# apple/ml-pgdvs

Measured on AMD Instinct MI355X. Metric: novel-view frames/s at 1080p x 24 src frames; achieved HBM GB/s vs gfx950 peak, higher is better.
Workload: dtype f32

## Files before the change

### ml-pgdvs_amd/csrc/fused.h

```cpp
#pragma once
#include "common.h"

namespace pgdvs {

struct WarpExtras {
  uint8_t *zero_a, *zero_b;
  uint4 *zero0, *zero1, *zero2, *zero3;
  int n16_0, n16_1, n16_2, n16_3;
  int32_t *chunk_cnt;
};
int dyn_warp_fused(int H, int W, const float *dyn_mask1, const float *occ, int use_flow_consistency, const float *flow12,
                   const float *depth1, const float *depth2, const float *rgb1, const float *rgb2, const float *cam1,
                   const float *cam2, const float *times, uint8_t *mask_eff, uint8_t *valid, float *pcl, float *rgbf,
                   const WarpExtras &ex, hipStream_t st);

int compact_gather_bbox(const uint8_t *flags, int64_t n, const int32_t *chunk_cnt, int32_t *idx_out, int32_t *count_out,
                        const float *rows_in, float *rows_out, unsigned *bbox, int32_t *zero_per_row, int zero_mult, hipStream_t st);

void knn_grid_state_block(void *workspace, int64_t capacity, void **block, int64_t *bytes, unsigned **bbox, void **tab,
                          int64_t *tab_bytes, int32_t **occ_count, int *occ_mult, void **coarse, int64_t *coarse_bytes);
int knn_grid_mean_dist_prepared(const float *pts, const int32_t *count, int64_t capacity, int K, float *avg_out, void *workspace,
                                int64_t workspace_bytes, hipStream_t st);

void outlier_hist_block(void *workspace, void **block, int64_t *bytes);
int outlier_keep_fused(const float *avg, const int32_t *count, int64_t capacity, float std_thres, float *thres_out,
                       const int32_t *idx, uint8_t *keep, void *workspace, int64_t workspace_bytes, hipStream_t st);

int dyn_splat_scatter_part_fused(int H, int W, const float *rgb1, const float *rgb2, const float *flow12, const float *cam_tgt,
                                 const float *pcl, const uint8_t *keep, float *flow_1_to_tgt, float *valid_mask,
                                 const float *noise, const unsigned long long *rng, float alpha, void *workspace,
                                 bool flags_cleared, hipStream_t st);
uint8_t *dyn_splat_flag_map(void *workspace, int H, int W);


void raster_counter_block(void *workspace, int64_t n_rows, int H, int W, float radius, void **block, int64_t *bytes);
int points_raster_bounded_cleared(const float *pts, int64_t pts_stride, const float *feat, int64_t feat_stride, int64_t n_points,
                                  const int64_t *n_points_dev, int64_t row_bound, int32_t *status_dev, const float *cam_tgt,
                                  float radius, int K, int H, int W, float *rgb, int rgb_planar, float *mask, void *workspace,
                                  int64_t workspace_bytes, pgdvs_stream_t stream, bool counters_cleared);

}
```

### ml-pgdvs_amd/csrc/raster.hip

```cpp
#include <cstdlib>

#include "common.h"
#include "raster_cam.h"
#include "wave.h"

namespace pgdvs {

constexpr int kTile = 16;

struct TileBox {
  int tx0, tx1, ty0, ty1;
};

__device__ __forceinline__ TileBox tile_box(const RasterCam &rc, float3 p, float radius, int H,
                                            int W, int ntx, int nty) {
  TileBox b;
  b.tx0 = 1;
  b.tx1 = 0;
  b.ty0 = 1;
  b.ty1 = 0;
  if (!(p.z >= 0.0f) || !isfinite(p.x) || !isfinite(p.y)) return b;
  float offx = rc.range_x / 2.0f, offy = rc.range_y / 2.0f;
  float xc = (float)(W - 1) - ((p.x + offx) * (float)W - offx) / rc.range_x;
  float yc = (float)(H - 1) - ((p.y + offy) * (float)H - offy) / rc.range_y;
  float rpx = radius * (float)W / rc.range_x + 0.0625f;
  float rpy = radius * (float)H / rc.range_y + 0.0625f;
  float x0 = ceilf(xc - rpx), x1 = floorf(xc + rpx);
  float y0 = ceilf(yc - rpy), y1 = floorf(yc + rpy);
  if (x1 < x0 || y1 < y0) return b;
  if (x1 < 0.0f || y1 < 0.0f || x0 > (float)(W - 1) || y0 > (float)(H - 1)) return b;
  int ix0 = x0 < 0.0f ? 0 : (int)x0, iy0 = y0 < 0.0f ? 0 : (int)y0;
  int ix1 = x1 > (float)(W - 1) ? W - 1 : (int)x1, iy1 = y1 > (float)(H - 1) ? H - 1 : (int)y1;
  b.tx0 = ix0 / kTile;
  b.tx1 = ix1 / kTile;
  b.ty0 = iy0 / kTile;
  b.ty1 = iy1 / kTile;
// ... 131 lines not shown
    b.tx0 = 1; b.tx1 = 0; b.ty0 = 1; b.ty1 = 0;
    float pz = 0.0f;
    if (i < n) {
      float3 p = point_to_ndc(rc, cur[0], cur[1], cur[2]);
      b = tile_box(rc, p, radius, H, W, ntx, nty);
      pz = p.z + 0.0f;
    }
    int nx = 2, ny = 2;
    if (!box2) {
      nx = wave_max_i32_scalar(b.tx1 - b.tx0 + 1);
      ny = wave_max_i32_scalar(b.ty1 - b.ty0 + 1);
    }
    for (int jy = 0; jy < ny; ++jy)
      for (int jx = 0; jx < nx; ++jx) {
        int tx = b.tx0 + jx, ty = b.ty0 + jy;
        int t = (tx <= b.tx1 && ty <= b.ty1) ? ty * ntx + tx : -1;
        if (tile_bound != nullptr && t >= 0 && pz > tile_bound[t]) t = -1;
        if (local)
          wave_tile_count_lds(s_tab, t);
        else
          wave_tile_count(tile_count, t);
      }
  }
  if (local) {
    __syncthreads();
    for (int t = threadIdx.x; t < ntiles; t += kBinThreads) {
      const int v = s_tab[t];
      if (v) __hip_atomic_fetch_add(&tile_count[t], v, __ATOMIC_RELAXED, __HIP_MEMORY_SCOPE_AGENT);
    }
  }
}

__global__ void __launch_bounds__(1024)
raster_scan_kernel(const int32_t *__restrict__ counts, int n, int32_t *__restrict__ offsets, const int32_t *__restrict__ run_flag) {
  __shared__ int wave_sums[1024 / kWave];
  if (run_flag != nullptr && *run_flag == 0) return;
  constexpr int kPer = 8;
  const int lane = threadIdx.x & 63, wave = threadIdx.x >> 6;
  int carry = 0;
  for (int start = 0; start < n; start += 1024 * kPer) {
    const int i0 = start + (int)threadIdx.x * kPer;
    int v[kPer], s = 0;
#pragma unroll
    for (int k = 0; k < kPer; ++k) {
      v[k] = i0 + k < n ? counts[i0 + k] : 0;
      s += v[k];
    }
    const int x = wave_incl_scan(s);
    if (lane == 63) wave_sums[wave] = x;
    __syncthreads();
    int run = carry + x - s, total = 0;
#pragma unroll
    for (int w = 0; w < 1024 / kWave; ++w) {
      if (w < wave) run += wave_sums[w];
      total += wave_sums[w];
    }
#pragma unroll
    for (int k = 0; k < kPer; ++k) {
      if (i0 + k < n) offsets[i0 + k] = run;
      run += v[k];
    }
    carry += total;
    __syncthreads();
  }
  if (threadIdx.x == 0) offsets[n] = carry;
}

constexpr int kFillPer = 4;
// ... 211 lines not shown
#pragma unroll
    for (int k = 0; k < K - 1; ++k) c[k] = kk < key[k];
    c[K - 1] = true;
#pragma unroll
    for (int k = K - 1; k > 0; --k) key[k] = c[k - 1] ? key[k - 1] : (c[k] ? kk : key[k]);
    key[0] = c[0] ? kk : key[0];
  }
};

constexpr int kSortCap = 2048;
constexpr int kSortCapLong = 4096;
constexpr int kSortBuckets = 1024;
constexpr int kSortMaxBucket = 64;

template <int K>
__device__ __forceinline__ void rank_insert(float (&key)[K], float r) {
#pragma unroll
  for (int k = K - 1; k > 0; --k) key[k] = __builtin_amdgcn_fmed3f(key[k - 1], key[k], r);
  asm("v_min_f32 %0, %1, %2" : "=v"(key[0]) : "v"(key[0]), "v"(r));
}

__device__ __forceinline__ float readlane_f(float v, int lane) {
  return __int_as_float(__builtin_amdgcn_readlane(__float_as_int(v), lane));
}

template <int K, int kCap, bool kFrag>
__global__ void __launch_bounds__(256, kCap <= kSortCap ? (kFrag ? 4 : 5) : 2)
raster_tile_kernel(const float4 *__restrict__ lists, const int32_t *__restrict__ offsets, int64_t list_capacity,
                   const float4 *__restrict__ seg_lists, const int32_t *__restrict__ seg_count, int seg,
                   const int32_t *__restrict__ seg_overflow, int pass,
                   const float *__restrict__ feat, int64_t feat_stride, float radius, int H, int W,
                   int ntx, int nty, int tiles_per_xcd, int64_t *__restrict__ idx_out,
                   float *__restrict__ zbuf_out, float *__restrict__ dist_out,
                   float *__restrict__ rgb_out, int rgb_planar, float *__restrict__ mask_out, int32_t *__restrict__ stats) {
  constexpr int kSortPerThread = kCap / 256;
  __shared__ uint2 s_buf[kCap];
  uint2 *s_kz = s_buf;
  float2 *s_xy = reinterpret_cast<float2 *>(s_buf);
  __shared__ unsigned s_id[kCap];
  __shared__ unsigned s_zr[kFrag ? kCap : 1];
  __shared__ float4 s_wave[4][68];
  unsigned *s_cnt = reinterpret_cast<unsigned *>(&s_wave[0][0]);
  static_assert(kSortBuckets * 4 <= 4 * 68 * 16, "the counters alias the strips");
  static_assert(kCap * (kFrag ? 16 : 12) + 4 * 68 * 16 + 128 <= (kCap <= kSortCap ? (kFrag ? 40960 : 32768) : 81920),
                "four / five (two) workgroups per CU");
  static_assert(kCap % 256 == 0 && kCap <= 4096, "every thread owns kCap / 256 entries; positions are packed in 12 bits");
  __shared__ unsigned s_red[12];
  __shared__ int s_flag;
  const int ntiles = ntx * nty;
  (void)tiles_per_xcd;
  const int tile = blockIdx.x;
  if (tile >= ntiles) return;
  const int ty = tile / ntx, tx = tile - ty * ntx;
  const int tid = threadIdx.x, lane = tid & 63, wave = tid >> 6;
  const int lx = (wave & 1) * 8 + (lane & 7), ly = (wave >> 1) * 8 + (lane >> 3);
  const int xi = tx * kTile + lx, yi = ty * kTile + ly;
  const bool inside = xi < W && yi < H;
  const float range_x = W > H ? 2.0f * (float)W / (float)H : 2.0f;
  const float range_y = H > W ? 2.0f * (float)H / (float)W : 2.0f;
  const float xf = inside ? pix_to_ndc(W - 1 - xi, W, range_x) : __builtin_nanf("");
  const float yf = pix_to_ndc(H - 1 - yi, H, range_y);
  const float r2 = radius * radius;
  const int qx0 = tx * kTile + (wave & 1) * 8, qy0 = ty * kTile + (wave >> 1) * 8;
  const float margin = radius * 1.001f + 1e-6f;
  const float bx_hi = pix_to_ndc(W - 1 - qx0, W, range_x) + margin;
  const float bx_lo = pix_to_ndc(W - 1 - (qx0 + 7), W, range_x) - margin;
  const float by_hi = pix_to_ndc(H - 1 - qy0, H, range_y) + margin;
// ... 272 lines not shown
  const size_t pix = (size_t)yi * W + xi;
  float t = 0.0f;
#pragma unroll
  for (int k = 0; k < K; ++k)
    if (has[k]) t = t + (1.0f - rd2[k] / r2);
  t = t > 1e-4f ? t : 1e-4f;
  float acc[3] = {0.f, 0.f, 0.f}, ones = 0.0f;
#pragma unroll
  for (int k = 0; k < K; ++k) {
    if (idx_out) idx_out[pix * K + k] = has[k] ? (int64_t)rid[k] : (int64_t)-1;
    if (zbuf_out) zbuf_out[pix * K + k] = has[k] ? rz[k] : -1.0f;
    if (dist_out) dist_out[pix * K + k] = rd2[k];
    if (has[k]) {
      float w = 1.0f - rd2[k] / r2;
      ones = ones + w * 1.0f / t;
      if (rgb_out) {
        const float *f = feat + (int64_t)rid[k] * feat_stride;
#pragma unroll
        for (int c = 0; c < 3; ++c) acc[c] = acc[c] + w * f[c] / t;
      }
    }
  }
  if (rgb_out) {
    if (rgb_planar) {
      const size_t P = (size_t)H * W;
#pragma unroll
      for (int c = 0; c < 3; ++c) rgb_out[c * P + pix] = acc[c];
    } else {
#pragma unroll
      for (int c = 0; c < 3; ++c) rgb_out[pix * 3 + c] = acc[c];
    }
  }
  if (mask_out) mask_out[pix] = ones > 0.0f ? 1.0f : 0.0f;
}

__global__ void raster_status_kernel(const int64_t *__restrict__ n_dev, int32_t *__restrict__ status) {
  if (threadIdx.x == 0) *status = (n_dev && *n_dev > 0) ? 1 : ((n_dev && *n_dev < 0) ? 2 : 0);
}

static int64_t max_tiles_per_point(float radius, int H, int W) {
  float range_x = W > H ? 2.0f * (float)W / (float)H : 2.0f;
  float range_y = H > W ? 2.0f * (float)H / (float)W : 2.0f;
  double wx = 2.0 * ((double)radius * W / range_x + 1.5) + 2.0;
  double wy = 2.0 * ((double)radius * H / range_y + 1.5) + 2.0;
  int64_t nx = (int64_t)(wx / kTile) + 2, ny = (int64_t)(wy / kTile) + 2;
  int64_t ntx = cdiv(W, kTile), nty = cdiv(H, kTile);
  if (nx > ntx) nx = ntx;
  if (ny > nty) ny = nty;
  return nx * ny;
}

constexpr double kSegLayoutDensity = 2.2;
constexpr int kSegEntries = 4096;
struct RasterWs {
  int32_t *tile_count, *cursor, *offsets;
  int32_t *seg_cursor;
  float4 *seg_lists;
  int seg_entries;
  int32_t *stats;
  unsigned *zmin;
  float *tile_bound;
  float4 *lists;
  int64_t list_capacity;
  int64_t total_bytes;
};

// ... 53 lines not shown
    for (int w = 0; w < 16; ++w) {
      m = s_max[w] > m ? s_max[w] : m;
      l += s_long[w];
      tt += s_tot[w];
    }
    out[0] = tt;
    out[1] = m;
    out[2] = l;
    out[3] = stats[0];
  }
}

void raster_counters(const void *workspace, int64_t n_rows, int H, int W, float radius, int64_t *out_dev, hipStream_t st) {
  const RasterWs ws = raster_ws_layout(const_cast<void *>(workspace), n_rows, H, W, radius);
  const int ntiles = (int)(cdiv(W, kTile) * cdiv(H, kTile));
  PGDVS_LAUNCH("raster_counters", raster_counters_kernel, dim3(1), dim3(1024), 0, st, (const int32_t *)ws.offsets, ntiles,
               (const int32_t *)ws.stats, out_dev, (const int32_t *)ws.seg_cursor, ws.seg_entries);
}

}

using namespace pgdvs;

namespace pgdvs {
void raster_counter_block(void *workspace, int64_t n_rows, int H, int W, float radius, void **block, int64_t *bytes) {
  const RasterWs ws = raster_ws_layout(workspace, n_rows, H, W, radius);
  *block = ws.tile_count;
  *bytes = (int64_t)((char *)ws.offsets - (char *)ws.tile_count);
}
}
static int points_raster_impl(const float *pts, int64_t pts_stride, const float *feat, int64_t feat_stride, int64_t n_points,
                              const int64_t *n_points_dev, int32_t *status_dev, const float *cam_tgt, float radius, int K,
                              int H, int W, int64_t *idx, float *zbuf, float *dist2, float *rgb, int rgb_planar, float *mask,
                              void *workspace, int64_t workspace_bytes, pgdvs_stream_t stream, bool counters_cleared);
namespace pgdvs {
int points_raster_bounded_cleared(const float *pts, int64_t pts_stride, const float *feat, int64_t feat_stride, int64_t n_points,
                                  const int64_t *n_points_dev, int64_t row_bound, int32_t *status_dev, const float *cam_tgt,
                                  float radius, int K, int H, int W, float *rgb, int rgb_planar, float *mask, void *workspace,
                                  int64_t workspace_bytes, pgdvs_stream_t stream, bool counters_cleared) {
  PGDVS_REQUIRE(row_bound >= 0 && status_dev && n_points >= 0, "points_raster_bounded_cleared: bad arguments");
  if (n_points_dev == nullptr && n_points > row_bound) {
    set_error("pgdvs_points_raster_bounded: %lld rows given (host count) but the row bound is %lld", (long long)n_points,
              (long long)row_bound);
    return PGDVS_ERR_INVALID;
  }
  return points_raster_impl(pts, pts_stride, feat, feat_stride, n_points < row_bound ? n_points : row_bound, n_points_dev,
                            status_dev, cam_tgt, radius, K, H, W, nullptr, nullptr, nullptr, rgb, rgb_planar, mask, workspace,
                            workspace_bytes, stream, counters_cleared);
}
}

PGDVS_API int64_t pgdvs_points_raster_workspace_bytes(int64_t n_points, int H, int W, float radius) {
  if (n_points < 0 || H <= 0 || W <= 0) return -1;
  const RasterWs w = raster_ws_layout(nullptr, n_points, H, W, radius);
  if (w.list_capacity >= (1ll << 31)) {
    set_error("pgdvs_points_raster: %lld points x this radius exceeds the 2^31 tile-list entries supported", (long long)n_points);
    return PGDVS_ERR_UNSUPPORTED;
  }
  return w.total_bytes;
}

template <int K>
static void launch_tile(dim3 grid, hipStream_t st, const RasterWs &ws, const float *feat,
                        int64_t feat_stride, float radius, int H, int W, int ntx, int nty,
                        int tiles_per_xcd, int64_t *idx, float *zbuf, float *dist2, float *rgb,
                        int rgb_planar, float *mask, bool long_lists, int seg) {
  const float4 *sl = (const float4 *)ws.seg_lists;
  const int32_t *sc = (const int32_t *)ws.seg_cursor, *so = (const int32_t *)(ws.stats + 1);
  if (zbuf != nullptr) {
    PGDVS_LAUNCH("raster_tile", (raster_tile_kernel<K, kSortCap, true>), grid, dim3(256), 0, st, (const float4 *)ws.lists,
                 (const int32_t *)ws.offsets, ws.list_capacity, sl, sc, seg, so, long_lists ? 1 : 0, feat, feat_stride, radius, H, W, ntx, nty,
                 tiles_per_xcd, idx, zbuf, dist2, rgb, rgb_planar, mask, ws.stats);
  } else {
    PGDVS_LAUNCH("raster_tile", (raster_tile_kernel<K, kSortCap, false>), grid, dim3(256), 0, st, (const float4 *)ws.lists,
                 (const int32_t *)ws.offsets, ws.list_capacity, sl, sc, seg, so, long_lists ? 1 : 0, feat, feat_stride, radius, H, W, ntx, nty,
                 tiles_per_xcd, idx, zbuf, dist2, rgb, rgb_planar, mask, ws.stats);
  }
  if (long_lists) {
    PGDVS_LAUNCH("raster_tile_long", (raster_tile_kernel<K, kSortCapLong, true>), grid, dim3(256), 0, st, (const float4 *)ws.lists,
                 (const int32_t *)ws.offsets, ws.list_capacity, sl, sc, seg, so, 2, feat, feat_stride, radius, H, W, ntx, nty, tiles_per_xcd, idx, zbuf,
                 dist2, rgb, rgb_planar, mask, ws.stats);
  }
}

static int points_raster_impl(const float *pts, int64_t pts_stride, const float *feat, int64_t feat_stride, int64_t n_points,
                              const int64_t *n_points_dev, int32_t *status_dev, const float *cam_tgt, float radius, int K,
                              int H, int W, int64_t *idx, float *zbuf, float *dist2, float *rgb, int rgb_planar, float *mask,
                              void *workspace, int64_t workspace_bytes, pgdvs_stream_t stream, bool counters_cleared = false);

PGDVS_API int pgdvs_points_raster(const float *pts, int64_t pts_stride, const float *feat,
                                  int64_t feat_stride, int64_t n_points,
                                  const int64_t *n_points_dev, const float *cam_tgt, float radius,
                                  int K, int H, int W, int64_t *idx, float *zbuf, float *dist2,
                                  float *rgb, int rgb_planar, float *mask, void *workspace,
                                  int64_t workspace_bytes, pgdvs_stream_t stream) {
  return points_raster_impl(pts, pts_stride, feat, feat_stride, n_points, n_points_dev, nullptr, cam_tgt, radius, K, H, W, idx,
                            zbuf, dist2, rgb, rgb_planar, mask, workspace, workspace_bytes, stream);
}

PGDVS_API int pgdvs_points_raster_bounded(const float *pts, int64_t pts_stride, const float *feat, int64_t feat_stride,
                                          int64_t n_points, const int64_t *n_points_dev, int64_t row_bound,
                                          int32_t *status_dev, const float *cam_tgt, float radius, int K, int H, int W,
                                          int64_t *idx, float *zbuf, float *dist2, float *rgb, int rgb_planar, float *mask,
                                          void *workspace, int64_t workspace_bytes, pgdvs_stream_t stream) {
  PGDVS_REQUIRE(row_bound >= 0 && status_dev, "pgdvs_points_raster_bounded: bad row_bound / null status_dev");
  PGDVS_REQUIRE(n_points >= 0, "pgdvs_points_raster_bounded: bad n_points");
  if (n_points_dev == nullptr && n_points > row_bound) {
    set_error("pgdvs_points_raster_bounded: %lld rows given (host count) but the row bound is %lld", (long long)n_points,
              (long long)row_bound);
    return PGDVS_ERR_INVALID;
  }
  return points_raster_impl(pts, pts_stride, feat, feat_stride, n_points < row_bound ? n_points : row_bound, n_points_dev,
                            status_dev, cam_tgt, radius, K, H, W, idx, zbuf, dist2, rgb, rgb_planar, mask, workspace,
                            workspace_bytes, stream);
}

static int points_raster_impl(const float *pts, int64_t pts_stride, const float *feat, int64_t feat_stride, int64_t n_points,
                              const int64_t *n_points_dev, int32_t *status_dev, const float *cam_tgt, float radius, int K,
                              int H, int W, int64_t *idx, float *zbuf, float *dist2, float *rgb, int rgb_planar, float *mask,
                              void *workspace, int64_t workspace_bytes, pgdvs_stream_t stream, bool counters_cleared) {
  PGDVS_REQUIRE(H > 0 && W > 0 && (int64_t)H * W < (1ll << 31), "pgdvs_points_raster: bad H/W");
  PGDVS_REQUIRE(n_points >= 0 && n_points < (1ll << 31), "pgdvs_points_raster: bad n_points");
  PGDVS_REQUIRE(cam_tgt && (n_points == 0 || pts) && pts_stride >= 3, "pgdvs_points_raster: bad points");
  PGDVS_REQUIRE(!rgb || n_points == 0 || (feat && feat_stride >= 3), "pgdvs_points_raster: rgb output needs features");
  PGDVS_REQUIRE(radius > 0.0f, "pgdvs_points_raster: radius must be > 0");
  if (K < 1 || K > kRasterMaxK) {
    set_error("pgdvs_points_raster: points_per_pixel must be in [1, %d]", kRasterMaxK);
    return PGDVS_ERR_UNSUPPORTED;
  }
  RasterWs ws = raster_ws_layout(workspace, n_points, H, W, radius);
  if (ws.list_capacity >= (1ll << 31)) {
    set_error("pgdvs_points_raster: %lld points x %lld tiles per point exceeds the 2^31 tile-list entries supported",
              (long long)n_points, (long long)(ws.list_capacity / (n_points > 0 ? n_points : 1)));
    return PGDVS_ERR_UNSUPPORTED;
  }
  if (!workspace || workspace_bytes < ws.total_bytes) {
    set_error("pgdvs_points_raster: workspace too small (%lld < %lld)", (long long)workspace_bytes,
              (long long)ws.total_bytes);
    return PGDVS_ERR_WORKSPACE;
  }
  hipStream_t st = as_stream(stream);
  const int ntx = (int)cdiv(W, kTile), nty = (int)cdiv(H, kTile), ntiles = ntx * nty;
  if (!counters_cleared) {
    hipError_t e = hipMemsetAsync(ws.tile_count, 0, (size_t)((char *)ws.offsets - (char *)ws.tile_count), st);
    if (e != hipSuccess) {
      set_error("points_raster memset: %s", hipGetErrorString(e));
      return PGDVS_ERR_LAUNCH;
    }
  }
  const bool small_table = ntiles <= kBinSlots / 2;
  const float *tile_bound = nullptr;
  int64_t gate_rows = 0;
  {
// ... 18 lines not shown
      }
      tile_bound = ws.tile_bound;
    }
  }
  if (n_points == 0 && status_dev != nullptr) {
    PGDVS_LAUNCH("raster_status", raster_status_kernel, dim3(1), dim3(64), 0, st, n_points_dev, status_dev);
  }
  const int seg = (n_points > 0 && n_points < gate_rows && ws.seg_lists != nullptr) ? ws.seg_entries : 0;
  const int32_t *run_flag = seg > 0 ? ws.stats + 1 : nullptr;
  const int64_t fill_chunks = cdiv(n_points, (int64_t)kFillThreads * kFillPer);
  const unsigned g_fill = (unsigned)(fill_chunks < 4096 ? fill_chunks : 4096);
  if (seg > 0) {
    if (small_table) {
      PGDVS_LAUNCH("raster_fill", raster_fill_kernel<kBinSlots / 2>, dim3(g_fill), dim3(kFillThreads), 0, st, pts, pts_stride, n_points, n_points_dev,
                   cam_tgt, radius, H, W, ntx, nty, (const int32_t *)nullptr, ws.seg_cursor, ws.seg_lists, ws.list_capacity, tile_bound, gate_rows,
                   seg, ws.stats + 1, status_dev, (const int32_t *)nullptr);
    } else {
      PGDVS_LAUNCH("raster_fill", raster_fill_kernel<kBinSlots>, dim3(g_fill), dim3(kFillThreads), 0, st, pts, pts_stride, n_points, n_points_dev,
                   cam_tgt, radius, H, W, ntx, nty, (const int32_t *)nullptr, ws.seg_cursor, ws.seg_lists, ws.list_capacity, tile_bound, gate_rows,
                   seg, ws.stats + 1, status_dev, (const int32_t *)nullptr);
    }
  }
  if (n_points > 0) {
    unsigned g = (unsigned)(cdiv(n_points, kBinThreads) < 512 ? cdiv(n_points, kBinThreads) : 512);
    if (seg > 0 && g > 256) g = 256;
    if (small_table) {
      PGDVS_LAUNCH(seg > 0 ? "raster_exact_count" : "raster_project_count", raster_project_count_kernel<kBinSlots / 2>, dim3(g), dim3(kBinThreads), 0, st, pts,
                   pts_stride, n_points, n_points_dev, cam_tgt, radius, H, W, ntx, nty, ws.tile_count, status_dev, tile_bound, gate_rows, run_flag);
    } else {
      PGDVS_LAUNCH(seg > 0 ? "raster_exact_count" : "raster_project_count", raster_project_count_kernel<kBinSlots>, dim3(g), dim3(kBinThreads), 0, st, pts,
                   pts_stride, n_points, n_points_dev, cam_tgt, radius, H, W, ntx, nty, ws.tile_count, status_dev, tile_bound, gate_rows, run_flag);
    }
  }
  PGDVS_LAUNCH(seg > 0 ? "raster_exact_scan" : "raster_scan", raster_scan_kernel, dim3(1), dim3(1024), 0, st, ws.tile_count, ntiles, ws.offsets, run_flag);
  if (n_points > 0) {
    const unsigned g_exact_fill = seg > 0 && g_fill > 256 ? 256u : g_fill;
    if (small_table) {
      PGDVS_LAUNCH(seg > 0 ? "raster_exact_fill" : "raster_fill", raster_fill_kernel<kBinSlots / 2>, dim3(g_exact_fill), dim3(kFillThreads), 0, st, pts, pts_stride, n_points, n_points_dev, cam_tgt,
                   radius, H, W, ntx, nty, (const int32_t *)ws.offsets, ws.cursor, ws.lists, ws.list_capacity, tile_bound, gate_rows,
                   0, (int32_t *)nullptr, (int32_t *)nullptr, run_flag);
    } else {
      PGDVS_LAUNCH(seg > 0 ? "raster_exact_fill" : "raster_fill", raster_fill_kernel<kBinSlots>, dim3(g_exact_fill), dim3(kFillThreads), 0, st, pts, pts_stride, n_points, n_points_dev, cam_tgt,
                   radius, H, W, ntx, nty, (const int32_t *)ws.offsets, ws.cursor, ws.lists, ws.list_capacity, tile_bound, gate_rows,
                   0, (int32_t *)nullptr, (int32_t *)nullptr, run_flag);
    }
  }
  const int tiles_per_xcd = (int)cdiv(ntiles, 8);
  dim3 grid((unsigned)ntiles);
  const bool long_lists = n_points > 0 && n_points >= gate_rows;
#define PGDVS_TILE_CASE(KK)                                                                      \
  case KK:                                                                                       \
    launch_tile<KK>(grid, st, ws, feat, feat_stride, radius, H, W, ntx, nty, tiles_per_xcd, idx, \
                    zbuf, dist2, rgb, rgb_planar, mask, long_lists, seg);                        \
    break;
  switch (K) {
    PGDVS_TILE_CASE(1)
    PGDVS_TILE_CASE(2)
    PGDVS_TILE_CASE(3)
    PGDVS_TILE_CASE(4)
    PGDVS_TILE_CASE(5)
    PGDVS_TILE_CASE(6)
    PGDVS_TILE_CASE(7)
    PGDVS_TILE_CASE(8)
  }
#undef PGDVS_TILE_CASE
  return check_launch("points_raster");
}
```

### ml-pgdvs_amd/csrc/softsplat.hip

```cpp
#include "common.h"
#include "fused.h"
#include "wave.h"

namespace pgdvs {

__device__ __forceinline__ void atomic_add_f32(float *p, float v) {
  __hip_atomic_fetch_add(p, v, __ATOMIC_RELAXED, __HIP_MEMORY_SCOPE_AGENT);
}

template <int kN>
__device__ __forceinline__ void lds_add_f32(uint32_t *const (&cell)[kN], const float (&add)[kN], const bool (&on)[kN]) {
  uint32_t seen[kN], want[kN];
#pragma unroll
  for (int i = 0; i < kN; ++i)
    if (on[i]) seen[i] = __hip_atomic_load(cell[i], __ATOMIC_RELAXED, __HIP_MEMORY_SCOPE_WORKGROUP);
  bool again = false;
#pragma unroll
  for (int i = 0; i < kN; ++i)
    if (on[i]) {
      want[i] = seen[i];
      seen[i] = atomicCAS(cell[i], want[i], __float_as_uint(__uint_as_float(want[i]) + add[i]));
    }
#pragma unroll
  for (int i = 0; i < kN; ++i) again = again || (on[i] && seen[i] != want[i]);
  if (again) {
#pragma unroll
    for (int i = 0; i < kN; ++i)
      if (on[i])
        while (seen[i] != want[i]) {
          want[i] = seen[i];
          seen[i] = atomicCAS(cell[i], want[i], __float_as_uint(__uint_as_float(want[i]) + add[i]));
        }
  }
}
// ... 294 lines not shown
#pragma unroll
      for (int pl = 0; pl < 5; ++pl) {
        const float v = val[pl];
        const bool skip = (pl == 4 && me == 0.0f) || (c.w[k] == 0.0f && isfinite(v));
        add[pl] = v * c.w[k];
        on[pl] = in_win && !skip;
        cell[pl] = reinterpret_cast<uint32_t *>(&s_acc[pl][in_win ? wy * kSplatWin + wx : 0]);
        if (!in_win && !skip) atomic_add_f32(acc + (size_t)pl * P + c.idx[k], add[pl]);
      }
      lds_add_f32(cell, add, on);
    }
  }
  __syncthreads();
  for (int i = threadIdx.x; i < kSplatWin * kSplatWin; i += 256) {
    const int ty = oy + i / kSplatWin, tx = ox + i % kSplatWin;
    if (tx >= W || ty >= H) continue;
#pragma unroll
    for (int pl = 0; pl < 5; ++pl) {
      const float v = s_acc[pl][i];
      if (v != 0.0f) atomic_add_f32(acc + (size_t)pl * P + (size_t)ty * W + tx, v);
    }
  }
}

__global__ void __launch_bounds__(256)
dyn_splat_finish_kernel(int P, const float *__restrict__ acc, const uint8_t *__restrict__ flags,
                        const float *__restrict__ static_rgb,
                        float *__restrict__ dyn_rgb, float *__restrict__ dyn_mask,
                        float *__restrict__ comb, float *__restrict__ comb_st,
                        float *__restrict__ comb_dy, unsigned long long *__restrict__ rng) {
  int p = blockIdx.x * blockDim.x + threadIdx.x;
  if (p >= P) return;
  if (p == 0 && rng != nullptr) rng[1] = rng[1] + 1ull;
  const bool live = flags[p] != 0;
  float nrm = live ? acc[(size_t)3 * P + p] + 0.0000001f : 1.0f;
  float mk = live ? acc[(size_t)4 * P + p] / nrm : 0.0f;
  float dm = mk > 1e-3f ? 1.0f : 0.0f;
  dyn_mask[p] = dm;
#pragma unroll
  for (int k = 0; k < 3; ++k) {
    float v = live ? (acc[(size_t)k * P + p] / nrm) * dm : 0.0f;
    dyn_rgb[(size_t)k * P + p] = v;
    if (static_rgb) {
      float a = (1.0f - dm) * static_rgb[(size_t)k * P + p];
      float b = dm * v;
      if (comb_st) comb_st[(size_t)k * P + p] = a;
      if (comb_dy) comb_dy[(size_t)k * P + p] = b;
      if (comb) comb[(size_t)k * P + p] = a + b;
    }
  }
}

__global__ void __launch_bounds__(256)
softsplat_bwd_kernel(const float *__restrict__ in, const float *__restrict__ flow,
                     const float *__restrict__ outgrad, float *__restrict__ ingrad,
                     float *__restrict__ flowgrad, int C, int H, int W) {
  const int64_t P = (int64_t)H * W;
  const int64_t p = (int64_t)blockIdx.x * blockDim.x + threadIdx.x;
  if (p >= P) return;
  const int n = blockIdx.y;
  const int y = (int)(p / W), x = (int)(p - (int64_t)y * W);
  const float X = (float)x + flow[((int64_t)n * 2 + 0) * P + p];
  const float Y = (float)y + flow[((int64_t)n * 2 + 1) * P + p];
  bool ok = isfinite(X) && isfinite(Y);
  const float flx = floorf(X), fly = floorf(Y);
  if (ok && (flx < -2.0f || flx > (float)W || fly < -2.0f || fly > (float)H)) ok = false;
  const int nwx = ok ? (int)flx : -8, nwy = ok ? (int)fly : -8;
  const int cx[4] = {nwx, nwx + 1, nwx, nwx + 1}, cy[4] = {nwy, nwy, nwy + 1, nwy + 1};
  const float sex = (float)(nwx + 1), sey = (float)(nwy + 1), wx = (float)nwx, wy = (float)nwy;
  const float w[4] = {(sex - X) * (sey - Y), (X - wx) * (sey - Y), (sex - X) * (Y - wy), (X - wx) * (Y - wy)};
  const float dx[4] = {-1.0f * (sey - Y), +1.0f * (sey - Y), -1.0f * (Y - wy), +1.0f * (Y - wy)};
  const float dy[4] = {(sex - X) * -1.0f, (X - wx) * -1.0f, (sex - X) * +1.0f, (X - wx) * +1.0f};
  bool inb[4];
  int64_t off[4];
#pragma unroll
  for (int k = 0; k < 4; ++k) {
    inb[k] = ok && cx[k] >= 0 && cx[k] < W && cy[k] >= 0 && cy[k] < H;
    off[k] = inb[k] ? (int64_t)cy[k] * W + cx[k] : 0;
  }
  float gfx = 0.0f, gfy = 0.0f;
  for (int ch = 0; ch < C; ++ch) {
    const float *og = outgrad + ((int64_t)n * C + ch) * P;
    const float v = in[((int64_t)n * C + ch) * P + p];
// ... 214 lines not shown
```

### ml-pgdvs_amd/csrc/view_geo.cpp

```cpp
#include <chrono>
#include <condition_variable>
#include <cstring>
#include <functional>
#include <thread>
#include <map>
#include <mutex>
#include <vector>

#include "common.h"
#include "fused.h"
#include "scan.h"

namespace pgdvs {

int view_prep(const float *flat_tgt, const float *flat_src, const float *time_src, const float *time_tgt, float *blocks,
              float *times, hipStream_t st);

int static_aggregate_for_view(const float *rgbs, const float *depths, const uint8_t *dyn_masks, const double *K3s_host,
                              const double *c2ws_host, int S, int H, int W, float *out, float *xyz_out, int64_t capacity,
                              int64_t *count_out, void *workspace, int64_t workspace_bytes, pgdvs_stream_t stream,
                              bool params_cached, void *zero_extra, int64_t zero_extra_bytes);

int dyn_splat_scatter_part(int H, int W, const float *rgb1, const float *rgb2, const float *flow12, const float *flow_1_to_tgt,
                           const float *valid_dyn_mask_1, const float *noise, const unsigned long long *rng, float alpha,
                           void *workspace, hipStream_t st);
int dyn_splat_finish_part(int H, int W, unsigned long long *rng, const float *static_rgb, float *render_dyn_rgb,
                          float *render_dyn_mask, float *combined, float *combined_static, float *combined_dyn, void *workspace,
                          hipStream_t st);

void raster_counters(const void *workspace, int64_t n_rows, int H, int W, float radius, int64_t *out_dev, hipStream_t st);
void knn_grid_counter_words(const void *workspace, int64_t capacity, int64_t qcapacity, const int32_t **to_ring,
                            const int32_t **to_coarse, const int32_t **to_exhaustive);
const unsigned *agg_stat_words(const void *workspace, int S, int H, int W, int64_t capacity);

__global__ void view_counters_kernel(const int64_t *__restrict__ static_rows, int64_t static_rows_host,
                                     const int32_t *__restrict__ knn_queries, const int32_t *__restrict__ to_ring,
                                     const int32_t *__restrict__ to_coarse, const int32_t *__restrict__ to_exhaustive,
                                     const unsigned *__restrict__ agg_stat, int64_t *__restrict__ out) {
  if (threadIdx.x != 0) return;
  out[PGDVS_VIEW_CNT_STATIC_ROWS] = static_rows ? *static_rows : static_rows_host;
  out[PGDVS_VIEW_CNT_KNN_QUERIES] = knn_queries ? *knn_queries : 0;
  out[PGDVS_VIEW_CNT_KNN_TO_RING] = to_ring ? *to_ring : 0;
  out[PGDVS_VIEW_CNT_KNN_TO_COARSE] = to_coarse ? *to_coarse : 0;
  out[PGDVS_VIEW_CNT_KNN_TO_EXHAUSTIVE] = to_exhaustive ? *to_exhaustive : 0;
  int64_t queued = 0;
  if (agg_stat)
    for (int k = 1; k <= 64; ++k) queued += agg_stat[k];
  out[PGDVS_VIEW_CNT_AGG_FP64_POINTS] = queued;
  out[PGDVS_VIEW_CNT_AGG_REFERENCE_ORDER] = agg_stat ? agg_stat[0] : 0;
  for (int k = PGDVS_VIEW_CNT_AGG_REFERENCE_ORDER + 1; k < PGDVS_VIEW_COUNTERS; ++k) out[k] = 0;
}

namespace {

struct ViewWs {
  float *cams;
  float *times;
  void *agg;
  int64_t agg_bytes;
  void *raster;
  int64_t raster_bytes;
// ... 190 lines not shown
  int occ_mult = 0;
  if (d.remove_outlier) {
    ex.zero_a = w.keep;
    ex.chunk_cnt = w.chunk_cnt;
    void *blk = nullptr, *tab = nullptr, *coarse = nullptr;
    int64_t bytes = 0, tab_bytes = 0, coarse_bytes = 0;
    knn_grid_state_block(w.knn, P, &blk, &bytes, &bbox, &tab, &tab_bytes, &occ_count, &occ_mult, &coarse, &coarse_bytes);
    ex.zero3 = reinterpret_cast<uint4 *>(coarse);
    ex.n16_3 = (int)(coarse_bytes / 16);
    ex.zero0 = reinterpret_cast<uint4 *>(blk);
    ex.n16_0 = (int)(bytes / 16);
    ex.zero2 = reinterpret_cast<uint4 *>(tab);
    ex.n16_2 = (int)(tab_bytes / 16);
    outlier_hist_block(w.outlier, &blk, &bytes);
    ex.zero1 = reinterpret_cast<uint4 *>(blk);
    ex.n16_1 = (int)(bytes / 16);
  }
  PGDVS_REQUIRE(d.dyn_mask1 && d.flow12 && d.depth1 && d.depth2 && d.rgb1 && d.rgb2, "pgdvs_view_geo_forward: null input pointer");
  VG_TRY(dyn_warp_fused(H, W, d.dyn_mask1, d.flow_occ, d.use_flow_consistency, d.flow12, d.depth1, d.depth2, d.rgb1, d.rgb2, cam1,
                        cam2, w.times, nullptr, w.valid, w.pcl, nullptr, ex, st));
  const uint8_t *keep = w.valid;
  if (d.remove_outlier) {
    VG_TRY(compact_gather_bbox(w.valid, P, w.chunk_cnt, w.idx, w.cnt, w.pcl, w.pts, bbox, occ_count, occ_mult, st));
    VG_TRY(knn_grid_mean_dist_prepared(w.pts, w.cnt, P, d.outlier_knn, w.avg, w.knn, w.knn_bytes, st));
    VG_TRY(outlier_keep_fused(w.avg, w.cnt, P, d.outlier_std_thres, w.thres, w.idx, w.keep, w.outlier, w.outlier_bytes, st));
    keep = w.keep;
  }
  const unsigned long long *rng = (d.noise == nullptr && d.rng_state != nullptr) ? reinterpret_cast<const unsigned long long *>(d.rng_state) : nullptr;
  VG_TRY(dyn_splat_scatter_part_fused(H, W, d.rgb1, d.rgb2, d.flow12, cam_t, w.pcl, keep, nullptr, nullptr, d.noise, rng, d.alpha,
                                      w.splat, true, st));
  return PGDVS_OK;
}

int view_forward(const pgdvs_view_geo_desc &d, void *workspace, int64_t workspace_bytes, pgdvs_stream_t stream) {
  PGDVS_REQUIRE(d.flat_cam_tgt && d.flat_cam_src && d.time_src && d.time_tgt && d.rgb1 && d.rgb2 && d.depth1 && d.depth2 &&
                    d.dyn_mask1 && d.flow12,
                "pgdvs_view_geo_forward: null input pointer");
  PGDVS_REQUIRE(d.static_rgb && d.static_mask && d.render_dyn_rgb && d.render_dyn_mask && d.combined && d.combined_static &&
                    d.combined_dyn && d.raster_status,
                "pgdvs_view_geo_forward: null output pointer");
  PGDVS_REQUIRE(!d.use_flow_consistency || d.flow_occ, "pgdvs_view_geo_forward: flow_occ required");
  PGDVS_REQUIRE(d.agg_S > 0 || d.st_rows == 0 || d.st_pcl_rgb, "pgdvs_view_geo_forward: no static cloud");
  PGDVS_REQUIRE(d.agg_S <= 0 || (d.agg_rgbs && d.agg_depths && d.agg_masks && d.agg_K3s_host && d.agg_c2ws_host &&
                                  d.agg_cloud_out && d.agg_xyz_out && d.agg_count_out && d.agg_capacity > 0),
                "pgdvs_view_geo_forward: incomplete aggregation arguments");
  PGDVS_REQUIRE(d.alpha >= 0.0f, "pgdvs_view_geo_forward: alpha must be >= 0");
  PGDVS_REQUIRE(!d.remove_outlier || (d.outlier_knn >= 1 && d.outlier_knn + 1 <= 64),
                "pgdvs_view_geo_forward: dyn_pcl_outlier_knn must be in [1, 63]");
  ViewWs w;
  VG_TRY(view_layout(d, workspace, w));
  if (!workspace || workspace_bytes < w.total_bytes) {
    set_error("pgdvs_view_geo_forward: workspace too small (%lld < %lld)", (long long)workspace_bytes, (long long)w.total_bytes);
    return PGDVS_ERR_WORKSPACE;
  }
  hipStream_t st = as_stream(stream);
  const int H = d.H, W = d.W;
  VG_TRY(view_prep(d.flat_cam_tgt, d.flat_cam_src, d.time_src, d.time_tgt, w.cams, w.times, st));
  hipStream_t side = as_stream(d.side_stream);
  const bool forked = side != nullptr && side != st;
  hipEvent_t ev_join = nullptr;
  if (forked) {
    hipEvent_t ev_fork = ev_get();
    hipError_t e = hipEventRecord(ev_fork, st);
    if (e == hipSuccess) e = hipStreamWaitEvent(side, ev_fork, 0);
    ev_put(ev_fork);
    if (e != hipSuccess) {
      set_error("pgdvs_view_geo_forward: fork onto the side stream: %s", hipGetErrorString(e));
      return PGDVS_ERR_LAUNCH;
    }
  } else {
    VG_TRY(dyn_geometry(d, w, stream));
  }
  const bool on_worker = forked && option_int(options().side_thread) != 0;
  if (on_worker) {
    int dev = 0;
    (void)hipGetDevice(&dev);
    const pgdvs_view_geo_desc *dp = &d;
    const ViewWs *wp = &w;
    side_worker().submit(dev, [dp, wp] { return dyn_geometry(*dp, *wp, dp->side_stream); });
  }
  const float *cloud = d.st_pcl_rgb, *xyz = d.st_pcl_xyz;
  const int64_t *count_dev = d.st_count_dev;
  int64_t rows = d.st_rows;
  int rc = PGDVS_OK;
  bool counters_cleared = false;
  if (d.agg_S > 0) {
    void *cblk = nullptr;
    int64_t cbytes = 0;
    raster_counter_block(w.raster, w.raster_rows, H, W, d.radius, &cblk, &cbytes);
    rc = static_aggregate_for_view(d.agg_rgbs, d.agg_depths, d.agg_masks, d.agg_K3s_host, d.agg_c2ws_host, d.agg_S, H, W,
                                   d.agg_cloud_out, d.agg_xyz_out, d.agg_capacity, d.agg_count_out, w.agg, w.agg_bytes, stream,
                                   d.agg_params_cached != 0, cblk, cbytes);
    counters_cleared = true;
    cloud = d.agg_cloud_out;
    xyz = d.agg_xyz_out;
    count_dev = d.agg_count_out;
    rows = d.agg_capacity;
  }
  if (rc == PGDVS_OK) {
    const float *pts = xyz ? xyz : cloud;
    const int64_t pts_stride = xyz ? 3 : 6;
    const float *feat = cloud ? cloud + 3 : nullptr;
    rc = points_raster_bounded_cleared(pts, pts_stride, feat, 6, rows, count_dev, w.raster_rows, d.raster_status, w.cams, d.radius,
                                       d.K, H, W, d.static_rgb, 1, d.static_mask, w.raster, w.raster_bytes, stream, counters_cleared);
  }
  if (forked) {
    const int rc_dyn = on_worker ? side_worker().wait() : dyn_geometry(d, w, d.side_stream);
    ev_join = ev_get();
    hipError_t e = hipEventRecord(ev_join, side);
    if (e == hipSuccess) e = hipStreamWaitEvent(st, ev_join, 0);
    ev_put(ev_join);
    if (rc == PGDVS_OK) rc = rc_dyn;
    if (e != hipSuccess && rc == PGDVS_OK) {
      set_error("pgdvs_view_geo_forward: join: %s", hipGetErrorString(e));
      rc = PGDVS_ERR_LAUNCH;
    }
  }
  VG_TRY(rc);
  unsigned long long *rng = (d.noise == nullptr && d.rng_state != nullptr) ? reinterpret_cast<unsigned long long *>(d.rng_state) : nullptr;
  return dyn_splat_finish_part(H, W, rng, d.static_rgb, d.render_dyn_rgb, d.render_dyn_mask, d.combined, d.combined_static,
                               d.combined_dyn, w.splat, st);
}

}
}

using namespace pgdvs;

PGDVS_API int64_t pgdvs_view_geo_desc_size(void) { return (int64_t)sizeof(pgdvs_view_geo_desc); }

PGDVS_API int64_t pgdvs_view_geo_workspace_bytes(const pgdvs_view_geo_desc *desc) {
  if (!desc) {
    set_error("pgdvs_view_geo_workspace_bytes: null description");
    return PGDVS_ERR_INVALID;
  }
  ViewWs w;
  const int rc = view_layout(*desc, nullptr, w);
  return rc != PGDVS_OK ? (int64_t)rc : w.total_bytes;
}

PGDVS_API int pgdvs_view_geo_forward(const pgdvs_view_geo_desc *desc, void *workspace, int64_t workspace_bytes,
                                     pgdvs_stream_t stream) {
  PGDVS_REQUIRE(desc, "pgdvs_view_geo_forward: null description");
  const auto t0 = std::chrono::steady_clock::now();
  const int rc = view_forward(*desc, workspace, workspace_bytes, stream);
  const double dt = std::chrono::duration<double>(std::chrono::steady_clock::now() - t0).count();
  {
    std::lock_guard<std::mutex> lk(g_stat_mu);
    g_stat_calls += 1;
    g_stat_seconds += dt;
  }
  return rc;
}

// ... 29 lines not shown
```

Before: 1300.

## Fuse dynamic splat finish into raster tile kernel epilogue

Moves the dynamic-splat finishing step (normalize the splat accumulators, build the dynamic mask, compose with the static render) into the epilogue of the raster tile kernel. The kernel now uses its in-register static RGB instead of re-reading it from HBM, and one kernel launch goes away. To make this possible, the side-stream join now runs right before the tile launch through a callback, and the tail parameters travel to the device through the scan kernel into the status block. The risk is that the join happens earlier, which may shorten the overlap with the static raster pre-passes, and the tile kernel gains extra epilogue work and register pressure.

```diff
diff --git a/ml-pgdvs_amd/csrc/fused.h b/ml-pgdvs_amd/csrc/fused.h
--- a/ml-pgdvs_amd/csrc/fused.h
+++ b/ml-pgdvs_amd/csrc/fused.h
@@ -1,5 +1,6 @@
 #pragma once
 #include "common.h"
+#include "splat_tail.h"
 
 namespace pgdvs {
 
@@ -34,9 +35,14 @@
 
 
 void raster_counter_block(void *workspace, int64_t n_rows, int H, int W, float radius, void **block, int64_t *bytes);
+struct RasterTailHook {
+  TileTail tail;
+  int (*before_tiles)(void *ctx);
+  void *ctx;
+};
 int points_raster_bounded_cleared(const float *pts, int64_t pts_stride, const float *feat, int64_t feat_stride, int64_t n_points,
                                   const int64_t *n_points_dev, int64_t row_bound, int32_t *status_dev, const float *cam_tgt,
                                   float radius, int K, int H, int W, float *rgb, int rgb_planar, float *mask, void *workspace,
-                                  int64_t workspace_bytes, pgdvs_stream_t stream, bool counters_cleared);
+                                  int64_t workspace_bytes, pgdvs_stream_t stream, bool counters_cleared, const RasterTailHook *tail);
 
 }
diff --git a/ml-pgdvs_amd/csrc/raster.hip b/ml-pgdvs_amd/csrc/raster.hip
--- a/ml-pgdvs_amd/csrc/raster.hip
+++ b/ml-pgdvs_amd/csrc/raster.hip
@@ -1,7 +1,9 @@
 #include <cstdlib>
 
 #include "common.h"
+#include "fused.h"
 #include "raster_cam.h"
+#include "splat_tail.h"
 #include "wave.h"
 
 namespace pgdvs {
@@ -199,8 +201,10 @@
 }
 
 __global__ void __launch_bounds__(1024)
-raster_scan_kernel(const int32_t *__restrict__ counts, int n, int32_t *__restrict__ offsets, const int32_t *__restrict__ run_flag) {
+raster_scan_kernel(const int32_t *__restrict__ counts, int n, int32_t *__restrict__ offsets, const int32_t *__restrict__ run_flag,
+                   const TileTail tail, TileTail *__restrict__ tail_out) {
   __shared__ int wave_sums[1024 / kWave];
+  if (tail_out != nullptr && threadIdx.x == 0) *tail_out = tail;
   if (run_flag != nullptr && *run_flag == 0) return;
   constexpr int kPer = 8;
   const int lane = threadIdx.x & 63, wave = threadIdx.x >> 6;
@@ -478,7 +482,8 @@
                    const float *__restrict__ feat, int64_t feat_stride, float radius, int H, int W,
                    int ntx, int nty, int tiles_per_xcd, int64_t *__restrict__ idx_out,
                    float *__restrict__ zbuf_out, float *__restrict__ dist_out,
-                   float *__restrict__ rgb_out, int rgb_planar, float *__restrict__ mask_out, int32_t *__restrict__ stats) {
+                   float *__restrict__ rgb_out, int rgb_planar, float *__restrict__ mask_out, int32_t *__restrict__ stats,
+                   const TileTail *__restrict__ tail_dev) {
   constexpr int kSortPerThread = kCap / 256;
   __shared__ uint2 s_buf[kCap];
   uint2 *s_kz = s_buf;
@@ -817,6 +822,12 @@
     }
   }
   if (mask_out) mask_out[pix] = ones > 0.0f ? 1.0f : 0.0f;
+  if (tail_dev != nullptr) {
+    const TileTail tail = *tail_dev;
+    if (tile == 0 && tid == 0 && tail.rng != nullptr) tail.rng[1] = tail.rng[1] + 1ull;
+    splat_finish_pixel(pix, (size_t)H * W, tail.acc, tail.flags, true, acc[0], acc[1], acc[2], tail.dyn_rgb, tail.dyn_mask,
+                       tail.comb, tail.comb_st, tail.comb_dy);
+  }
 }
 
 __global__ void raster_status_kernel(const int64_t *__restrict__ n_dev, int32_t *__restrict__ status) {
@@ -936,13 +947,16 @@
 static int points_raster_impl(const float *pts, int64_t pts_stride, const float *feat, int64_t feat_stride, int64_t n_points,
                               const int64_t *n_points_dev, int32_t *status_dev, const float *cam_tgt, float radius, int K,
                               int H, int W, int64_t *idx, float *zbuf, float *dist2, float *rgb, int rgb_planar, float *mask,
-                              void *workspace, int64_t workspace_bytes, pgdvs_stream_t stream, bool counters_cleared);
+                              void *workspace, int64_t workspace_bytes, pgdvs_stream_t stream, bool counters_cleared,
+                              const RasterTailHook *tail);
 namespace pgdvs {
 int points_raster_bounded_cleared(const float *pts, int64_t pts_stride, const float *feat, int64_t feat_stride, int64_t n_points,
                                   const int64_t *n_points_dev, int64_t row_bound, int32_t *status_dev, const float *cam_tgt,
                                   float radius, int K, int H, int W, float *rgb, int rgb_planar, float *mask, void *workspace,
-                                  int64_t workspace_bytes, pgdvs_stream_t stream, bool counters_cleared) {
+                                  int64_t workspace_bytes, pgdvs_stream_t stream, bool counters_cleared, const RasterTailHook *tail) {
   PGDVS_REQUIRE(row_bound >= 0 && status_dev && n_points >= 0, "points_raster_bounded_cleared: bad arguments");
+  PGDVS_REQUIRE(tail == nullptr || (rgb && rgb_planar && tail->tail.acc && tail->tail.flags && tail->tail.dyn_rgb && tail->tail.dyn_mask),
+                "points_raster_bounded_cleared: the tail needs the planar static image and its own outputs");
   if (n_points_dev == nullptr && n_points > row_bound) {
     set_error("pgdvs_points_raster_bounded: %lld rows given (host count) but the row bound is %lld", (long long)n_points,
               (long long)row_bound);
@@ -950,7 +964,7 @@
   }
   return points_raster_impl(pts, pts_stride, feat, feat_stride, n_points < row_bound ? n_points : row_bound, n_points_dev,
                             status_dev, cam_tgt, radius, K, H, W, nullptr, nullptr, nullptr, rgb, rgb_planar, mask, workspace,
-                            workspace_bytes, stream, counters_cleared);
+                            workspace_bytes, stream, counters_cleared, tail);
 }
 }
 
@@ -968,29 +982,30 @@
 static void launch_tile(dim3 grid, hipStream_t st, const RasterWs &ws, const float *feat,
                         int64_t feat_stride, float radius, int H, int W, int ntx, int nty,
                         int tiles_per_xcd, int64_t *idx, float *zbuf, float *dist2, float *rgb,
-                        int rgb_planar, float *mask, bool long_lists, int seg) {
+                        int rgb_planar, float *mask, bool long_lists, int seg, const TileTail *tail) {
   const float4 *sl = (const float4 *)ws.seg_lists;
   const int32_t *sc = (const int32_t *)ws.seg_cursor, *so = (const int32_t *)(ws.stats + 1);
   if (zbuf != nullptr) {
     PGDVS_LAUNCH("raster_tile", (raster_tile_kernel<K, kSortCap, true>), grid, dim3(256), 0, st, (const float4 *)ws.lists,
                  (const int32_t *)ws.offsets, ws.list_capacity, sl, sc, seg, so, long_lists ? 1 : 0, feat, feat_stride, radius, H, W, ntx, nty,
-                 tiles_per_xcd, idx, zbuf, dist2, rgb, rgb_planar, mask, ws.stats);
+                 tiles_per_xcd, idx, zbuf, dist2, rgb, rgb_planar, mask, ws.stats, tail);
   } else {
     PGDVS_LAUNCH("raster_tile", (raster_tile_kernel<K, kSortCap, false>), grid, dim3(256), 0, st, (const float4 *)ws.lists,
                  (const int32_t *)ws.offsets, ws.list_capacity, sl, sc, seg, so, long_lists ? 1 : 0, feat, feat_stride, radius, H, W, ntx, nty,
-                 tiles_per_xcd, idx, zbuf, dist2, rgb, rgb_planar, mask, ws.stats);
+                 tiles_per_xcd, idx, zbuf, dist2, rgb, rgb_planar, mask, ws.stats, tail);
   }
   if (long_lists) {
     PGDVS_LAUNCH("raster_tile_long", (raster_tile_kernel<K, kSortCapLong, true>), grid, dim3(256), 0, st, (const float4 *)ws.lists,
                  (const int32_t *)ws.offsets, ws.list_capacity, sl, sc, seg, so, 2, feat, feat_stride, radius, H, W, ntx, nty, tiles_per_xcd, idx, zbuf,
-                 dist2, rgb, rgb_planar, mask, ws.stats);
+                 dist2, rgb, rgb_planar, mask, ws.stats, tail);
   }
 }
 
 static int points_raster_impl(const float *pts, int64_t pts_stride, const float *feat, int64_t feat_stride, int64_t n_points,
                               const int64_t *n_points_dev, int32_t *status_dev, const float *cam_tgt, float radius, int K,
                               int H, int W, int64_t *idx, float *zbuf, float *dist2, float *rgb, int rgb_planar, float *mask,
-                              void *workspace, int64_t workspace_bytes, pgdvs_stream_t stream, bool counters_cleared = false);
+                              void *workspace, int64_t workspace_bytes, pgdvs_stream_t stream, bool counters_cleared = false,
+                              const RasterTailHook *tail = nullptr);
 
 PGDVS_API int pgdvs_points_raster(const float *pts, int64_t pts_stride, const float *feat,
                                   int64_t feat_stride, int64_t n_points,
@@ -1022,7 +1037,8 @@
 static int points_raster_impl(const float *pts, int64_t pts_stride, const float *feat, int64_t feat_stride, int64_t n_points,
                               const int64_t *n_points_dev, int32_t *status_dev, const float *cam_tgt, float radius, int K,
                               int H, int W, int64_t *idx, float *zbuf, float *dist2, float *rgb, int rgb_planar, float *mask,
-                              void *workspace, int64_t workspace_bytes, pgdvs_stream_t stream, bool counters_cleared) {
+                              void *workspace, int64_t workspace_bytes, pgdvs_stream_t stream, bool counters_cleared,
+                              const RasterTailHook *tail) {
   PGDVS_REQUIRE(H > 0 && W > 0 && (int64_t)H * W < (1ll << 31), "pgdvs_points_raster: bad H/W");
   PGDVS_REQUIRE(n_points >= 0 && n_points < (1ll << 31), "pgdvs_points_raster: bad n_points");
   PGDVS_REQUIRE(cam_tgt && (n_points == 0 || pts) && pts_stride >= 3, "pgdvs_points_raster: bad points");
@@ -1107,7 +1123,10 @@
                    pts_stride, n_points, n_points_dev, cam_tgt, radius, H, W, ntx, nty, ws.tile_count, status_dev, tile_bound, gate_rows, run_flag);
     }
   }
-  PGDVS_LAUNCH(seg > 0 ? "raster_exact_scan" : "raster_scan", raster_scan_kernel, dim3(1), dim3(1024), 0, st, ws.tile_count, ntiles, ws.offsets, run_flag);
+  static_assert(sizeof(TileTail) <= 32 * sizeof(int32_t) && alignof(TileTail) <= 8, "the tail's slot in the status block");
+  TileTail *tail_dev = tail != nullptr ? reinterpret_cast<TileTail *>(ws.stats + 32) : nullptr;
+  PGDVS_LAUNCH(seg > 0 ? "raster_exact_scan" : "raster_scan", raster_scan_kernel, dim3(1), dim3(1024), 0, st, ws.tile_count, ntiles, ws.offsets, run_flag,
+               tail != nullptr ? tail->tail : TileTail{}, tail_dev);
   if (n_points > 0) {
     const unsigned g_exact_fill = seg > 0 && g_fill > 256 ? 256u : g_fill;
     if (small_table) {
@@ -1123,10 +1142,14 @@
   const int tiles_per_xcd = (int)cdiv(ntiles, 8);
   dim3 grid((unsigned)ntiles);
   const bool long_lists = n_points > 0 && n_points >= gate_rows;
+  if (tail != nullptr && tail->before_tiles != nullptr) {
+    const int rc = tail->before_tiles(tail->ctx);
+    if (rc != PGDVS_OK) return rc;
+  }
 #define PGDVS_TILE_CASE(KK)                                                                      \
   case KK:                                                                                       \
     launch_tile<KK>(grid, st, ws, feat, feat_stride, radius, H, W, ntx, nty, tiles_per_xcd, idx, \
-                    zbuf, dist2, rgb, rgb_planar, mask, long_lists, seg);                        \
+                    zbuf, dist2, rgb, rgb_planar, mask, long_lists, seg, (const TileTail *)tail_dev);\
     break;
   switch (K) {
     PGDVS_TILE_CASE(1)
diff --git a/ml-pgdvs_amd/csrc/softsplat.hip b/ml-pgdvs_amd/csrc/softsplat.hip
--- a/ml-pgdvs_amd/csrc/softsplat.hip
+++ b/ml-pgdvs_amd/csrc/softsplat.hip
@@ -1,5 +1,6 @@
 #include "common.h"
 #include "fused.h"
+#include "splat_tail.h"
 #include "wave.h"
 
 namespace pgdvs {
@@ -360,23 +361,13 @@
   int p = blockIdx.x * blockDim.x + threadIdx.x;
   if (p >= P) return;
   if (p == 0 && rng != nullptr) rng[1] = rng[1] + 1ull;
-  const bool live = flags[p] != 0;
-  float nrm = live ? acc[(size_t)3 * P + p] + 0.0000001f : 1.0f;
-  float mk = live ? acc[(size_t)4 * P + p] / nrm : 0.0f;
-  float dm = mk > 1e-3f ? 1.0f : 0.0f;
-  dyn_mask[p] = dm;
-#pragma unroll
-  for (int k = 0; k < 3; ++k) {
-    float v = live ? (acc[(size_t)k * P + p] / nrm) * dm : 0.0f;
-    dyn_rgb[(size_t)k * P + p] = v;
-    if (static_rgb) {
-      float a = (1.0f - dm) * static_rgb[(size_t)k * P + p];
-      float b = dm * v;
-      if (comb_st) comb_st[(size_t)k * P + p] = a;
-      if (comb_dy) comb_dy[(size_t)k * P + p] = b;
-      if (comb) comb[(size_t)k * P + p] = a + b;
-    }
-  }
+  float s[3] = {0.0f, 0.0f, 0.0f};
+  if (static_rgb) {
+#pragma unroll
+    for (int k = 0; k < 3; ++k) s[k] = static_rgb[(size_t)k * P + p];
+  }
+  splat_finish_pixel((size_t)p, (size_t)P, acc, flags, static_rgb != nullptr, s[0], s[1], s[2], dyn_rgb, dyn_mask, comb, comb_st,
+                     comb_dy);
 }
 
 __global__ void __launch_bounds__(256)
diff --git a/ml-pgdvs_amd/csrc/splat_tail.h b/ml-pgdvs_amd/csrc/splat_tail.h
--- /dev/null
+++ b/ml-pgdvs_amd/csrc/splat_tail.h
@@ -0,0 +1,39 @@
+#pragma once
+#include "common.h"
+
+namespace pgdvs {
+
+struct TileTail {
+  const float *acc;
+  const uint8_t *flags;
+  float *dyn_rgb, *dyn_mask;
+  float *comb, *comb_st, *comb_dy;
+  unsigned long long *rng;
+};
+
+__device__ __forceinline__ void splat_finish_pixel(size_t p, size_t P, const float *__restrict__ acc,
+                                                   const uint8_t *__restrict__ flags, bool has_static, float s0, float s1,
+                                                   float s2, float *__restrict__ dyn_rgb, float *__restrict__ dyn_mask,
+                                                   float *__restrict__ comb, float *__restrict__ comb_st,
+                                                   float *__restrict__ comb_dy) {
+  const bool live = flags[p] != 0;
+  float nrm = live ? acc[(size_t)3 * P + p] + 0.0000001f : 1.0f;
+  float mk = live ? acc[(size_t)4 * P + p] / nrm : 0.0f;
+  float dm = mk > 1e-3f ? 1.0f : 0.0f;
+  dyn_mask[p] = dm;
+  const float s[3] = {s0, s1, s2};
+#pragma unroll
+  for (int k = 0; k < 3; ++k) {
+    float v = live ? (acc[(size_t)k * P + p] / nrm) * dm : 0.0f;
+    dyn_rgb[(size_t)k * P + p] = v;
+    if (has_static) {
+      float a = (1.0f - dm) * s[k];
+      float b = dm * v;
+      if (comb_st) comb_st[(size_t)k * P + p] = a;
+      if (comb_dy) comb_dy[(size_t)k * P + p] = b;
+      if (comb) comb[(size_t)k * P + p] = a + b;
+    }
+  }
+}
+
+}
diff --git a/ml-pgdvs_amd/csrc/view_geo.cpp b/ml-pgdvs_amd/csrc/view_geo.cpp
--- a/ml-pgdvs_amd/csrc/view_geo.cpp
+++ b/ml-pgdvs_amd/csrc/view_geo.cpp
@@ -20,13 +20,6 @@
                               const double *c2ws_host, int S, int H, int W, float *out, float *xyz_out, int64_t capacity,
                               int64_t *count_out, void *workspace, int64_t workspace_bytes, pgdvs_stream_t stream,
                               bool params_cached, void *zero_extra, int64_t zero_extra_bytes);
-
-int dyn_splat_scatter_part(int H, int W, const float *rgb1, const float *rgb2, const float *flow12, const float *flow_1_to_tgt,
-                           const float *valid_dyn_mask_1, const float *noise, const unsigned long long *rng, float alpha,
-                           void *workspace, hipStream_t st);
-int dyn_splat_finish_part(int H, int W, unsigned long long *rng, const float *static_rgb, float *render_dyn_rgb,
-                          float *render_dyn_mask, float *combined, float *combined_static, float *combined_dyn, void *workspace,
-                          hipStream_t st);
 
 void raster_counters(const void *workspace, int64_t n_rows, int H, int W, float radius, int64_t *out_dev, hipStream_t st);
 void knn_grid_counter_words(const void *workspace, int64_t capacity, int64_t qcapacity, const int32_t **to_ring,
@@ -283,6 +276,28 @@
   return PGDVS_OK;
 }
 
+struct SideJoin {
+  const pgdvs_view_geo_desc &d;
+  const ViewWs &w;
+  hipStream_t st, side;
+  bool forked, on_worker, done;
+  int run() {
+    done = true;
+    if (!forked) return PGDVS_OK;
+    int rc = on_worker ? side_worker().wait() : dyn_geometry(d, w, d.side_stream);
+    hipEvent_t ev_join = ev_get();
+    hipError_t e = hipEventRecord(ev_join, side);
+    if (e == hipSuccess) e = hipStreamWaitEvent(st, ev_join, 0);
+    ev_put(ev_join);
+    if (e != hipSuccess && rc == PGDVS_OK) {
+      set_error("pgdvs_view_geo_forward: join: %s", hipGetErrorString(e));
+      rc = PGDVS_ERR_LAUNCH;
+    }
+    return rc;
+  }
+  static int hook(void *self) { return static_cast<SideJoin *>(self)->run(); }
+};
+
 int view_forward(const pgdvs_view_geo_desc &d, void *workspace, int64_t workspace_bytes, pgdvs_stream_t stream) {
   PGDVS_REQUIRE(d.flat_cam_tgt && d.flat_cam_src && d.time_src && d.time_tgt && d.rgb1 && d.rgb2 && d.depth1 && d.depth2 &&
                     d.dyn_mask1 && d.flow12,
@@ -309,7 +324,6 @@
   VG_TRY(view_prep(d.flat_cam_tgt, d.flat_cam_src, d.time_src, d.time_tgt, w.cams, w.times, st));
   hipStream_t side = as_stream(d.side_stream);
   const bool forked = side != nullptr && side != st;
-  hipEvent_t ev_join = nullptr;
   if (forked) {
     hipEvent_t ev_fork = ev_get();
     hipError_t e = hipEventRecord(ev_fork, st);
@@ -348,29 +362,32 @@
     count_dev = d.agg_count_out;
     rows = d.agg_capacity;
   }
+  RasterTailHook hook;
+  memset(&hook, 0, sizeof(hook));
+  hook.tail.acc = reinterpret_cast<const float *>(w.splat);
+  hook.tail.flags = dyn_splat_flag_map(w.splat, H, W);
+  hook.tail.dyn_rgb = d.render_dyn_rgb;
+  hook.tail.dyn_mask = d.render_dyn_mask;
+  hook.tail.comb = d.combined;
+  hook.tail.comb_st = d.combined_static;
+  hook.tail.comb_dy = d.combined_dyn;
+  hook.tail.rng = (d.noise == nullptr && d.rng_state != nullptr) ? reinterpret_cast<unsigned long long *>(d.rng_state) : nullptr;
+  SideJoin join{d, w, st, side, forked, on_worker, false};
+  hook.before_tiles = &SideJoin::hook;
+  hook.ctx = &join;
   if (rc == PGDVS_OK) {
     const float *pts = xyz ? xyz : cloud;
     const int64_t pts_stride = xyz ? 3 : 6;
     const float *feat = cloud ? cloud + 3 : nullptr;
     rc = points_raster_bounded_cleared(pts, pts_stride, feat, 6, rows, count_dev, w.raster_rows, d.raster_status, w.cams, d.radius,
-                                       d.K, H, W, d.static_rgb, 1, d.static_mask, w.raster, w.raster_bytes, stream, counters_cleared);
-  }
-  if (forked) {
-    const int rc_dyn = on_worker ? side_worker().wait() : dyn_geometry(d, w, d.side_stream);
-    ev_join = ev_get();
-    hipError_t e = hipEventRecord(ev_join, side);
-    if (e == hipSuccess) e = hipStreamWaitEvent(st, ev_join, 0);
-    ev_put(ev_join);
-    if (rc == PGDVS_OK) rc = rc_dyn;
-    if (e != hipSuccess && rc == PGDVS_OK) {
-      set_error("pgdvs_view_geo_forward: join: %s", hipGetErrorString(e));
-      rc = PGDVS_ERR_LAUNCH;
-    }
-  }
-  VG_TRY(rc);
-  unsigned long long *rng = (d.noise == nullptr && d.rng_state != nullptr) ? reinterpret_cast<unsigned long long *>(d.rng_state) : nullptr;
-  return dyn_splat_finish_part(H, W, rng, d.static_rgb, d.render_dyn_rgb, d.render_dyn_mask, d.combined, d.combined_static,
-                               d.combined_dyn, w.splat, st);
+                                       d.K, H, W, d.static_rgb, 1, d.static_mask, w.raster, w.raster_bytes, stream, counters_cleared,
+                                       &hook);
+  }
+  if (!join.done) {
+    const int rc_join = join.run();
+    if (rc == PGDVS_OK) rc = rc_join;
+  }
+  return rc;
 }
 
 }
```

Measured after the change: 1298. No clear change (-0.1%).
